# Zeudon/sound-event-localization-detection

Hardware: AMD Instinct MI355X
Metric: training clips/sec (4ch FOA 60s@24kHz) (higher is better)
Workload: dtype bf16; 1 GPU; crnn FOA 4-ch 60s clips, bs=32 windows (BASELINE configs[1]); parallelism=dp1

## Files before the change

### include/seld_hip.h

```cpp
#ifndef SELD_HIP_H_
#define SELD_HIP_H_

#include <stdint.h>

#ifdef __cplusplus
extern "C" {
#endif

int seld_init(int device);
int seld_shutdown(void);
int seld_version(void);
const char* seld_last_error(void);

int seld_set_mel_filterbank(const float* fb_host);

int seld_set_window(const float* window_host);

int seld_default_tables(float* window960, float* fb481x64, int* mel_b0_64, float* mel_wd_24x64,
                        float* mel_wu_24x64);

int64_t seld_num_frames(int64_t L);

int seld_logmel_f32(const float* pcm, int64_t N, int64_t C, int64_t L, float* out, int layout, void* stream);
int seld_logmel_i16(const int16_t* pcm, int64_t N, int64_t C, int64_t L, float* out, int layout, void* stream);
// ... 82 lines not shown
int seld_sum_chunks(const void* partial, int in_is_bf16, int64_t chunks, int64_t count, void* out, int out_is_bf16,
                    void* stream);

int64_t seld_column_sums_blocks(int64_t rows, int64_t n_cols);
int seld_column_sums(const void* g, int in_is_bf16, int64_t rows, int64_t n_cols, float* partial, void* out, int out_is_bf16,
                     void* stream);

int seld_multi_sum_chunks(const void* const* partial, void* const* out, const int64_t* counts, const int32_t* chunks,
                          const int32_t* flags, int count, void* stream);
int seld_multi_column_sums_scratch(const int64_t* rows, const int64_t* n_cols, int count, int64_t* partial_floats);
int seld_multi_column_sums(const void* const* g, void* const* out, const int64_t* rows, const int64_t* n_cols,
                           const int32_t* flags, int count, float* partial, int64_t partial_floats, void* stream);

int seld_gru_dwhh_finish(const void* p_gi, const void* p_n, int in_is_bf16, int64_t chunks, int64_t H, void* dw_hh,
                         int out_is_bf16, void* stream);

int seld_conv_weight_flip_transpose(const void* w, int elem_bytes, int64_t O, int64_t I, void* wt, void* stream);

int seld_conv3x3_wgrad_supported(int64_t F, int64_t Cin, int64_t Cout);
int64_t seld_conv3x3_wgrad_workspace_floats(int64_t B, int64_t T, int64_t F, int64_t Cin, int64_t Cout);
int seld_conv3x3_wgrad(const void* x, const void* dy, int64_t B, int64_t T, int64_t F, int64_t Cin, int64_t Cout,
                       void* dw, int dw_is_bf16, float* workspace, void* stream);

int64_t seld_conv_tail_workspace_floats(int C);
int seld_conv_tail_forward(const void* x, const void* residual, int is_bf16, int64_t rows, int C, int pool,
                           const float* weight, const float* bias, float* running_mean, float* running_var,
                           float momentum, float eps, int training, void* y, float* mean_invstd, float* scale_shift,
                           float* workspace, void* stream);
int seld_conv_tail_backward(const void* x, const void* residual, const void* dy, int is_bf16, int64_t rows, int C,
                            int pool, const float* mean_invstd, const float* scale_shift, void* dx, void* dresidual,
                            float* dweight, float* dbias, float* workspace, void* stream);

int seld_dwconv1d(const void* x, int is_bf16, const float* weight, const float* bias, int64_t B, int64_t T, int D, int K,
                  int flip_taps, void* y, void* stream);
int64_t seld_dwconv1d_wgrad_rows(int64_t B, int64_t T);
int seld_dwconv1d_wgrad(const void* x, const void* dy, int is_bf16, int64_t B, int64_t T, int D, int K, float* partial,
                        void* stream);

int64_t seld_gru_tile_rows(void);
int seld_gru_forward(const void* gi, int is_bf16, const void* w_hh_bf16, const float* b_hn, int64_t B,
                     int64_t T, int64_t H, void* y, void* saved_tile, void* stream);

int seld_gru_backward(const void* dy_tile, const void* saved_tile, const void* y, int is_bf16,
                      const void* w_hh_t_bf16, int64_t tiles, int64_t T, int64_t H, void* dg_tile, float* dbias,
                      void* stream);

// ... 19 lines not shown
```

### sound-event-localization-detection_amd/config.py

```python
from pathlib import Path

_SR = 24000


class Config:
    BASE_PATH = Path(__file__).parent
    AUDIO_PATH = BASE_PATH / "foa_dev"
    METADATA_PATH = BASE_PATH / "metadata_dev"
    OUTPUT_PATH = BASE_PATH / "outputs"
    CHECKPOINT_PATH = BASE_PATH / "checkpoints"

    USE_FULL_DATASET = True
    TRAIN_AUDIO_FILE = "fold3_room21_mix001.wav"
    TRAIN_META_FILE = "fold3_room21_mix001.csv"
    TEST_AUDIO_FILE = "fold4_room23_mix001.wav"
    TEST_META_FILE = "fold4_room23_mix001.csv"

    STARSS22_CLASSES = dict(enumerate((
        "Female speech, woman speaking", "Male speech, man speaking", "Clapping", "Telephone",
        "Laughter", "Domestic sounds", "Walk, footsteps", "Door, open or close", "Music",
        "Musical instrument", "Water tap, faucet", "Bell", "Knock", "Background")))

    MODEL_TYPE = "resnet_conformer"
    NUM_CLASSES = 14
# ... 31 lines not shown
    MIN_DELTA = 1e-4

    SAVE_EVERY_N_EPOCHS = 5
    KEEP_LAST_N_CHECKPOINTS = 3

    SPECTROGRAM_N_FFT = int(0.04 * _SR)
    SPECTROGRAM_HOP_LENGTH = int(0.02 * _SR)
    N_MELS = 64
    SR = _SR

    WINDOW_LENGTH = int(5 * _SR)
    HOP_LENGTH = int(1 * _SR)

    I = None
    J = None
    GRID_CELL_DEGREES = 10

    AMP_DTYPE = "bf16"
    CHANNELS_LAST = True
    FUSED_LOSS = True
    FUSED_CONV_TAIL = True
    CONV_DGRAD_AS_FORWARD = True
    FUSED_CONV_WGRAD = True
    FUSED_DWCONV = "auto"
    CONV1X1_AS_GEMM = True
    FUSED_QKV = True
    FUSED_LAYERNORM = True
    OVERLAP_WEIGHT_GRADS = True
    FUSED_GRU = True
    DEVICE_FEED = True
    MASTER_WEIGHTS = True
    FUSED_ADAM_KERNEL = True
    GRAPH_STEP = True
    OVERLAP_ALLREDUCE = True
    ALLREDUCE_CUT_LEVELS = 2
    GRAD_REDUCE_DTYPE = "param"
    TUNED_GEMMS = True
    DDP_BUCKET_MB = 8
    SYNC_BATCHNORM = False
    SEED = None
    FEATURE_SET = "logmel"
    FEATURE_CACHE_DIR = None
    THREE_TERM_LOSS = False
    GAUSSIAN_AUGMENT = False
    GAUSSIAN_SIGMA_AZIMUTH = 5.0
    GAUSSIAN_SIGMA_ELEVATION = 5.0
# ... 18 lines not shown
```

### sound-event-localization-detection_amd/model_crnn.py

```python
import torch
import torch.nn as nn
import torch.nn.functional as F

from seld_layernorm import run_head
from seld_linear import SeldLinear
from seld_rnn import SeldGRU


class _Conv3x3(torch.autograd.Function):

    enabled = True
    fused_wgrad = True

    @staticmethod
    def forward(ctx, x, weight):
        cdt = torch.get_autocast_dtype("cuda") if torch.is_autocast_enabled() else x.dtype
        with torch.autocast(device_type="cuda", enabled=False):
            xc, wc = x.to(cdt), weight.to(cdt)
            y = F.conv2d(xc, wc, padding=1)
        ctx.save_for_backward(xc, wc)
        ctx.dtypes = (x.dtype, weight.dtype)
        ctx.after_cut = bool(x.is_leaf and x.requires_grad)
        return y

# ... 36 lines not shown
        return dx, dw if dw.dtype == w_dtype else dw.to(w_dtype)


def conv3x3(c, x):
    if (x.is_cuda and _Conv3x3.enabled and c.kernel_size == (3, 3) and c.stride == (1, 1) and c.padding == (1, 1)
            and c.dilation == (1, 1) and c.groups == 1 and c.bias is None and c.padding_mode == "zeros"
            and x.is_contiguous(memory_format=torch.channels_last) and torch.is_grad_enabled()
            and (x.requires_grad or c.weight.requires_grad)):
        return _Conv3x3.apply(x, c.weight)
    return c(x)


class ConvBlock(nn.Module):

    def __init__(self, in_channels, out_channels, kernel_size=(3, 3), stride=(1, 1), padding=(1, 1), pool_size=None):
        super().__init__()
        self.conv = nn.Conv2d(in_channels, out_channels, kernel_size=kernel_size, stride=stride,
                              padding=padding, bias=False)
        self.bn = nn.BatchNorm2d(out_channels)
        self.act = nn.ReLU(inplace=True)
        self.pool = nn.MaxPool2d(pool_size) if pool_size else None

    def forward(self, x):
        x = conv3x3(self.conv, x)
        if x.is_cuda:
            import seld_convtail
            if seld_convtail.applicable(self, x):
                return seld_convtail.conv_tail(self, x)
        x = self.act(self.bn(x))
        return x if self.pool is None else self.pool(x)


def build_cnn_encoder(n_channels, n_mels, cnn_channels, max_pools=4):
    blocks = nn.ModuleList()
    channels, freq = n_channels, n_mels
    for depth, width in enumerate(cnn_channels):
        pool = (1, 2) if depth < max_pools else None
        blocks.append(ConvBlock(channels, width, pool_size=pool))
        channels = width
        if pool:
            freq //= pool[1]
    return blocks, channels, freq


def run_cnn_blocks(blocks, x, inner_cut=True):
    x = x.permute(0, 2, 1, 3)
# ... 59 lines not shown
```

### sound-event-localization-detection_amd/seld_native.py

```python
from __future__ import annotations

import ctypes
import os
import threading
from pathlib import Path

import torch

_HERE = Path(__file__).resolve().parent
LIB_PATH = Path(os.environ["SELD_HIP_LIB"]).resolve() if os.environ.get("SELD_HIP_LIB") else _HERE / "libseld_hip.so"

N_FFT = 960
HOP = 480
N_BINS = 481
N_MELS = 64

_lock = threading.Lock()
_lib = None
_initialised_devices = set()

_i64 = ctypes.c_int64
_int = ctypes.c_int
_ptr = ctypes.c_void_p

# ... 44 lines not shown
    lib.seld_smr_loss_workspace_bytes.argtypes = [_i64, _i64]
    lib.seld_smr_loss.argtypes = [_ptr, _int, _ptr, _ptr, _i64, _int, _int, _int, ctypes.c_float, ctypes.c_float,
                                  ctypes.c_float, _ptr, _ptr, _ptr, _ptr]
    lib.seld_multi_cast.argtypes = [_ptr, _ptr, _ptr, _int, _int, _ptr]
    lib.seld_stream_delay.argtypes = [_i64, _ptr]
    lib.seld_gru_fold_bias.argtypes = [_ptr, _ptr, _i64, _ptr, _int, _ptr, _ptr]
    lib.seld_gru_bias_grads.argtypes = [_ptr, _i64, _i64, _ptr, _ptr, _ptr]
    lib.seld_sum_chunks.argtypes = [_ptr, _int, _i64, _i64, _ptr, _int, _ptr]
    lib.seld_gru_dwhh_finish.argtypes = [_ptr, _ptr, _int, _i64, _i64, _ptr, _int, _ptr]
    lib.seld_column_sums.argtypes = [_ptr, _int, _i64, _i64, _ptr, _ptr, _int, _ptr]
    _pp, _pi64, _pi32 = ctypes.POINTER(ctypes.c_void_p), ctypes.POINTER(ctypes.c_int64), ctypes.POINTER(ctypes.c_int32)
    _f = ctypes.c_float
    lib.seld_multi_adam.argtypes = [_pp, _pi32, _pp, _pp, _pp, _pp, _pi64, _int, _ptr, _ptr, _f, _f, _f, _f, _f, _ptr]
    lib.seld_multi_sum_chunks.argtypes = [_pp, _pp, _pi64, _pi32, _pi32, _int, _ptr]
    lib.seld_multi_column_sums_scratch.argtypes = [_pi64, _pi64, _int, _pi64]
    lib.seld_multi_column_sums.argtypes = [_pp, _pp, _pi64, _pi64, _pi32, _int, _ptr, _i64, _ptr]
    lib.seld_column_sums_blocks.argtypes = [_i64, _i64]
    lib.seld_column_sums_blocks.restype = ctypes.c_int64
    lib.seld_conv_weight_flip_transpose.argtypes = [_ptr, _int, _i64, _i64, _ptr, _ptr]
    lib.seld_conv3x3_wgrad_supported.argtypes = [_i64, _i64, _i64]
    lib.seld_conv3x3_wgrad_workspace_floats.restype = _i64
    lib.seld_conv3x3_wgrad_workspace_floats.argtypes = [_i64, _i64, _i64, _i64, _i64]
    lib.seld_conv3x3_wgrad.argtypes = [_ptr, _ptr, _i64, _i64, _i64, _i64, _i64, _ptr, _int, _ptr, _ptr]
    lib.seld_layernorm_supported.argtypes = [_i64]
    lib.seld_layernorm_workspace_floats.restype = _i64
    lib.seld_layernorm_workspace_floats.argtypes = [_i64, _i64]
    lib.seld_layernorm_forward.argtypes = [_ptr, _int, _i64, _i64, _ptr, _ptr, ctypes.c_float, _int, _ptr, _ptr, _ptr]
    lib.seld_layernorm_backward.argtypes = [_ptr, _ptr, _int, _i64, _i64, _ptr, _ptr, _ptr, _int, _ptr, _ptr, _ptr,
                                            _ptr, _ptr]
    lib.seld_conv_tail_workspace_floats.restype = _i64
    lib.seld_conv_tail_workspace_floats.argtypes = [_int]
    lib.seld_conv_tail_forward.argtypes = [_ptr, _ptr, _int, _i64, _int, _int, _ptr, _ptr, _ptr, _ptr, ctypes.c_float,
                                           ctypes.c_float, _int, _ptr, _ptr, _ptr, _ptr, _ptr]
    lib.seld_conv_tail_backward.argtypes = [_ptr, _ptr, _ptr, _int, _i64, _int, _int, _ptr, _ptr, _ptr, _ptr, _ptr, _ptr,
                                            _ptr, _ptr]
    lib.seld_dwconv1d.argtypes = [_ptr, _int, _ptr, _ptr, _i64, _i64, _int, _int, _int, _ptr, _ptr]
    lib.seld_dwconv1d_wgrad.argtypes = [_ptr, _ptr, _int, _i64, _i64, _int, _int, _ptr, _ptr]
    lib.seld_dwconv1d_wgrad_rows.argtypes = [_i64, _i64]
    lib.seld_dwconv1d_wgrad_rows.restype = ctypes.c_int64
    lib.seld_gru_to_tile.argtypes = [_ptr, _int, _i64, _i64, _int, _ptr, _ptr]
    lib.seld_gru_from_pair_tile.argtypes = [_ptr, _int, _i64, _i64, _ptr, _ptr, _ptr]
    lib.seld_gru_previous_state.argtypes = [_ptr, _int, _i64, _i64, _ptr, _ptr]
    lib.seld_gru_tile_rows.restype = _i64
    lib.seld_gru_tile_rows.argtypes = []
    lib.seld_gru_forward.argtypes = [_ptr, _int, _ptr, _ptr, _i64, _i64, _i64, _ptr, _ptr, _ptr]
    lib.seld_gru_backward.argtypes = [_ptr, _ptr, _ptr, _int, _ptr, _i64, _i64, _i64, _ptr, _ptr, _ptr]
# ... 794 lines not shown
            and dy.dtype == torch.bfloat16 and tuple(w.shape[2:]) == (3, 3)):
        return False
    b, cin, t, f = x.shape
    if tuple(dy.shape) != (b, w.shape[0], t, f) or w.shape[1] != cin:
        return False
    if not (x.is_contiguous(memory_format=torch.channels_last) and dy.is_contiguous(memory_format=torch.channels_last)
            and w.is_contiguous(memory_format=torch.channels_last)):
        return False
    return bool(load_library().seld_conv3x3_wgrad_supported(f, cin, w.shape[0]))


def conv3x3_wgrad(x: torch.Tensor, dy: torch.Tensor, dw: torch.Tensor) -> torch.Tensor:
    if not conv3x3_wgrad_applicable(x, dy, dw) or dw.dtype not in (torch.float32, torch.bfloat16):
        raise SeldNativeError("conv3x3_wgrad: unsupported shapes, dtypes or layouts")
    b, cin, t, f = x.shape
    cout = dy.shape[1]
    with _device_guard(ensure_init(x.device)):
        lib = load_library()
        ws = torch.empty(int(lib.seld_conv3x3_wgrad_workspace_floats(b, t, f, cin, cout)), dtype=torch.float32,
                         device=x.device)
        check(lib.seld_conv3x3_wgrad(_p(x), _p(dy), b, t, f, cin, cout, _p(dw), _is_bf16(dw), _p(ws),
                                     _stream_ptr(x.device)), "seld_conv3x3_wgrad")
    return dw



def _prep_pcm(pcm):
    squeeze = pcm.dim() == 2
    if squeeze:
        pcm = pcm.unsqueeze(0)
    if pcm.dim() != 3 or not pcm.is_cuda or pcm.dtype not in (torch.float32, torch.int16):
        raise SeldNativeError("pcm must be a GPU tensor [N, C, L] (or [C, L]) of float32 or int16")
    return pcm.contiguous(), squeeze


def stft(pcm: torch.Tensor) -> torch.Tensor:
    pcm, squeeze = _prep_pcm(pcm)
    n, c, length = pcm.shape
    index = ensure_init(pcm.device)
    out = torch.empty((n, c, num_frames(length), N_BINS, 2), dtype=torch.float32, device=pcm.device)
    fn = load_library().seld_stft_f32 if pcm.dtype == torch.float32 else load_library().seld_stft_i16
    with _device_guard(index):
        check(fn(_p(pcm), n, c, length, _p(out), _stream_ptr(pcm.device)), "seld_stft")
    spec = torch.view_as_complex(out)
    return spec[0] if squeeze else spec

# ... 51 lines not shown
```

### sound-event-localization-detection_amd/trainer.py

```python
import gc
import logging
import os
import random
from contextlib import nullcontext
from datetime import datetime
from pathlib import Path

import numpy as np
import torch
import torch.distributed as dist
from torch.utils.data import DataLoader, RandomSampler, SequentialSampler
from tqdm import tqdm

from config import Config
from dataset import SELDDataset
from loss import SMRSELDLoss
from model import SMRSELDWithCSPDarkNet
from model_conformer import SELD_Conformer
from model_crnn import SELD_CRNN
from resnet50_model import SELD_ResNet50_Conformer
from seld_rnn import SeldGRU
from utils import get_local_rank, get_rank, get_world_size, safe_torch_load
from visualization import plot_loss_curves, visualize_grid_predictions, visualize_loss_components

# ... 21 lines not shown
        logger.info("Initializing ResNet50-Conformer model...")
        return SELD_ResNet50_Conformer(n_mels=config.N_MELS, conf_d_model=config.RESNET_CONF_D_MODEL,
                                       conf_n_heads=config.RESNET_CONF_N_HEADS,
                                       conf_n_layers=config.RESNET_CONF_N_LAYERS,
                                       dropout=config.RESNET_DROPOUT, **common)
    logger.info("Initializing CSPDarkNet (CNN) model...")
    return SMRSELDWithCSPDarkNet(use_small=use_small_model, **common)


def prepare_model_for_device(model, device):
    model = model.to(device)
    if device.type == "cuda" and getattr(config, "CHANNELS_LAST", True):
        model = model.to(memory_format=torch.channels_last)
    SeldGRU.fused_enabled = bool(getattr(config, "FUSED_GRU", True))
    if device.type == "cuda":
        import seld_convtail
        import seld_gru
        seld_convtail.enabled = bool(getattr(config, "FUSED_CONV_TAIL", True))
        import model_crnn
        model_crnn._Conv3x3.enabled = bool(getattr(config, "CONV_DGRAD_AS_FORWARD", True)) and \
            os.environ.get("SELD_CONV_AS_FWD", "1") != "0"
        model_crnn._Conv3x3.fused_wgrad = bool(getattr(config, "FUSED_CONV_WGRAD", True)) and \
            os.environ.get("SELD_CONV_WGRAD", "1") != "0"
        if os.environ.get("SELD_DWCONV") is None:
            import seld_dwconv
            seld_dwconv.enabled = getattr(config, "FUSED_DWCONV", "auto")
            if seld_dwconv.enabled == "auto" and graph_step_enabled(device):
                seld_dwconv.enabled = True
        import seld_layernorm
        seld_layernorm.enabled = bool(getattr(config, "FUSED_LAYERNORM", True)) and \
            os.environ.get("SELD_LAYERNORM", "1") != "0"
        if os.environ.get("SELD_OVERLAP") is None:
            import seld_overlap
            seld_overlap.enabled = bool(getattr(config, "OVERLAP_WEIGHT_GRADS", True))
        import seld_linear
        seld_linear.conv1x1_as_gemm = bool(getattr(config, "CONV1X1_AS_GEMM", True)) and \
            os.environ.get("SELD_CONV1X1_GEMM", "1") != "0"
        import model_conformer
        model_conformer.MultiHeadSelfAttention.fused_qkv = bool(getattr(config, "FUSED_QKV", True)) and \
            os.environ.get("SELD_FUSED_QKV", "1") != "0"
        for module in model.modules():
            if isinstance(module, SeldGRU) and SeldGRU.fused_enabled:
                seld_gru.pack_parameters(module)
            if isinstance(module, model_conformer.MultiHeadSelfAttention):
                module.pack_parameters()
        if os.environ.get("SELD_CUT_LEVELS") is None:
# ... 696 lines not shown
```

Measured before the change: 154.8 clips/s.

## Fuse first CRNN conv block (conv3x3+BN+ReLU+pool) into MFMA kernels

Adds a dedicated HIP path for the first CRNN conv block, which has 4 input channels and 64 output channels. The forward pass recomputes the 3x3 convolution with MFMA in a stats pass and then an apply pass, so the full-resolution pre-pool activation is never written to memory. The backward pass likewise fuses dgrad-free weight gradients and BN gradients, since the input needs no grad. The cost is recomputing the conv twice per pass and extra launches for the statistics reduction.

```diff
diff --git a/include/seld_hip.h b/include/seld_hip.h
--- a/include/seld_hip.h
+++ b/include/seld_hip.h
@@ -128,6 +128,18 @@
 int seld_conv3x3_wgrad(const void* x, const void* dy, int64_t B, int64_t T, int64_t F, int64_t Cin, int64_t Cout,
                        void* dw, int dw_is_bf16, float* workspace, void* stream);
 
+int seld_convfirst_supported(int64_t F, int64_t Cin, int64_t Cout);
+int64_t seld_convfirst_workspace_floats(int backward);
+int seld_convfirst_forward(const void* in, const void* w, int w_is_bf16, int64_t w_sco, int64_t w_sci, int64_t w_sr,
+                           int64_t w_ss, int64_t B, int64_t T, int64_t F, const float* bn_weight, const float* bn_bias,
+                           float* running_mean, float* running_var, float momentum, float eps, void* y,
+                           float* mean_invstd, float* scale_shift, float* workspace, int phases, void* stream);
+int seld_convfirst_backward(const void* in, const void* w, int w_is_bf16, int64_t w_sco, int64_t w_sci, int64_t w_sr,
+                            int64_t w_ss, const void* dy, int64_t B, int64_t T, int64_t F, const float* mean_invstd,
+                            const float* scale_shift, void* dw, int dw_is_bf16, int64_t dw_sco, int64_t dw_sci,
+                            int64_t dw_sr, int64_t dw_ss, float* dgamma, float* dbeta, float* workspace, int phases,
+                            void* stream);
+
 int64_t seld_conv_tail_workspace_floats(int C);
 int seld_conv_tail_forward(const void* x, const void* residual, int is_bf16, int64_t rows, int C, int pool,
                            const float* weight, const float* bias, float* running_mean, float* running_var,
diff --git a/sound-event-localization-detection_amd/config.py b/sound-event-localization-detection_amd/config.py
--- a/sound-event-localization-detection_amd/config.py
+++ b/sound-event-localization-detection_amd/config.py
@@ -77,6 +77,7 @@
     FUSED_CONV_TAIL = True
     CONV_DGRAD_AS_FORWARD = True
     FUSED_CONV_WGRAD = True
+    FUSED_FIRST_BLOCK = True
     FUSED_DWCONV = "auto"
     CONV1X1_AS_GEMM = True
     FUSED_QKV = True
diff --git a/sound-event-localization-detection_amd/csrc/convfirst.hip b/sound-event-localization-detection_amd/csrc/convfirst.hip
--- /dev/null
+++ b/sound-event-localization-detection_amd/csrc/convfirst.hip
@@ -0,0 +1,711 @@
+#include <hip/hip_bf16.h>
+
+#include "seld_common.h"
+
+namespace seld {
+
+namespace {
+
+typedef __attribute__((ext_vector_type(8))) __bf16 bf16x8;
+typedef __attribute__((ext_vector_type(2))) __bf16 bf16x2;
+typedef __attribute__((ext_vector_type(2))) float f32x2;
+typedef __attribute__((ext_vector_type(4))) float f32x4;
+typedef __attribute__((ext_vector_type(4))) unsigned u32x4;
+typedef __attribute__((ext_vector_type(2))) short s16x2;
+typedef __attribute__((ext_vector_type(4))) short s16x4;
+typedef __attribute__((ext_vector_type(8))) short s16x8;
+typedef __attribute__((address_space(3))) s16x4 lds_s16x4;
+
+constexpr int kCfThreads = 256;
+constexpr int kCfPos = 256;
+constexpr int kCfTiles = kCfPos / 16;
+constexpr int kCfCout = 64;
+constexpr int kCfCin = 4;
+constexpr int kCfK = 36;
+constexpr int kCfMaxGroups = 512;
+constexpr int kCfImage = 3 * 258;
+constexpr int kCfStage = 3;
+constexpr int kCfSumThreads = 256;
+constexpr int kCfSumRows = 16;
+
+struct CfGeom {
+  int T, logF, chunks_per_clip, chunks;
+  long rows;
+};
+
+struct CfWeights {
+  const void* w;
+  int is_bf16;
+  int packed;
+  long sco, sci, sr, ss;
+};
+
+__device__ __forceinline__ unsigned pack_bf16_pair(float lo, float hi) {
+  const f32x2 v = {lo, hi};
+  return __builtin_bit_cast(unsigned, __builtin_convertvector(v, bf16x2));
+}
+__device__ __forceinline__ float round_bf16(float z) { return __uint_as_float(pack_bf16_pair(z, 0.0f) << 16); }
+__device__ __forceinline__ float bf16_lo(unsigned w) { return __uint_as_float(w << 16); }
+__device__ __forceinline__ float bf16_hi(unsigned w) { return __uint_as_float(w & 0xffff0000u); }
+
+__device__ __forceinline__ float cf_weight(const CfWeights& w, int co, int tap, int ci) {
+  const long i = co * w.sco + ci * w.sci + (tap / 3) * w.sr + (tap % 3) * w.ss;
+  if (w.is_bf16) return __uint_as_float(static_cast<unsigned>(static_cast<const unsigned short*>(w.w)[i]) << 16);
+  return round_bf16(static_cast<const float*>(w.w)[i]);
+}
+
+__device__ __forceinline__ void cf_load_weights(const CfWeights& w, int lane, bf16x8 (&wb)[4][2]) {
+  const int g = lane >> 4, c = lane & 15;
+  if (w.packed) {
+#pragma unroll
+    for (int nt = 0; nt < 4; ++nt) {
+      const uint2* const row = reinterpret_cast<const uint2*>(static_cast<const unsigned short*>(w.w) + (4 * c + nt) * kCfK);
+      const uint2 lo = row[2 * g], hi = row[2 * g + 1];
+      uint2 last = row[8];
+      if (g != 0) last = make_uint2(0u, 0u);
+      const u32x4 p0 = {lo.x, lo.y, hi.x, hi.y}, p1 = {last.x, last.y, 0u, 0u};
+      wb[nt][0] = __builtin_bit_cast(bf16x8, p0);
+      wb[nt][1] = __builtin_bit_cast(bf16x8, p1);
+    }
+    return;
+  }
+#pragma unroll
+  for (int nt = 0; nt < 4; ++nt) {
+    const int co = 4 * c + nt;
+    float v0[8], v1[8];
+#pragma unroll
+    for (int e = 0; e < 8; ++e) {
+      v0[e] = cf_weight(w, co, 2 * g + (e >> 2), e & 3);
+      v1[e] = (g == 0 && e < 4) ? cf_weight(w, co, 8, e & 3) : 0.0f;
+    }
+    const u32x4 p0 = {pack_bf16_pair(v0[0], v0[1]), pack_bf16_pair(v0[2], v0[3]), pack_bf16_pair(v0[4], v0[5]),
+                      pack_bf16_pair(v0[6], v0[7])};
+    const u32x4 p1 = {pack_bf16_pair(v1[0], v1[1]), pack_bf16_pair(v1[2], v1[3]), pack_bf16_pair(v1[4], v1[5]),
+                      pack_bf16_pair(v1[6], v1[7])};
+    wb[nt][0] = __builtin_bit_cast(bf16x8, p0);
+    wb[nt][1] = __builtin_bit_cast(bf16x8, p1);
+  }
+}
+
+__device__ __forceinline__ int cf_tap_shift(int tap, int W) { return (tap / 3 - 1) * W + tap % 3 - 1; }
+
+__device__ __forceinline__ int cf_image_row(int pos, int logF) {
+  const int F = 1 << logF;
+  return ((pos >> logF) + 1) * (F + 2) + (pos & (F - 1)) + 1;
+}
+
+struct CfLane {
+  int xr[kCfTiles / 4];
+  int row[kCfTiles / 4];
+  int pooled[kCfTiles / 4];
+  int sh0, sh1, sh8;
+  bool g0;
+};
+
+__device__ __forceinline__ CfLane cf_lane(int logF, int lane, int wave) {
+  CfLane ln;
+  const int W = (1 << logF) + 2, g = lane >> 4;
+#pragma unroll
+  for (int i = 0; i < kCfTiles / 4; ++i) {
+    const int pos = (wave + 4 * i) * 16;
+    ln.xr[i] = cf_image_row(pos + (lane & 15), logF);
+    ln.row[i] = pos >> logF;
+    ln.pooled[i] = ((pos + 4 * g) >> 1) * kCfCout + 4 * (lane & 15);
+  }
+  ln.sh0 = cf_tap_shift(2 * g, W);
+  ln.sh1 = cf_tap_shift(2 * g + 1, W);
+  ln.sh8 = W + 1;
+  ln.g0 = g == 0;
+  return ln;
+}
+
+__device__ __forceinline__ void cf_conv_tile(const uint2* img, const CfLane& ln, int i, const bf16x8 (&wb)[4][2],
+                                             unsigned (&xp)[4][2]) {
+  const int xr = ln.xr[i];
+  const uint2 t0 = img[xr + ln.sh0], t1 = img[xr + ln.sh1];
+  uint2 t8 = img[xr + ln.sh8];
+  if (!ln.g0) t8 = make_uint2(0u, 0u);
+  const u32x4 p0 = {t0.x, t0.y, t1.x, t1.y}, p1 = {t8.x, t8.y, 0u, 0u};
+  const bf16x8 a0 = __builtin_bit_cast(bf16x8, p0), a1 = __builtin_bit_cast(bf16x8, p1);
+#pragma unroll
+  for (int nt = 0; nt < 4; ++nt) {
+    f32x4 acc = {0.0f, 0.0f, 0.0f, 0.0f};
+    acc = __builtin_amdgcn_mfma_f32_16x16x32_bf16(a0, wb[nt][0], acc, 0, 0, 0);
+    acc = __builtin_amdgcn_mfma_f32_16x16x32_bf16(a1, wb[nt][1], acc, 0, 0, 0);
+    xp[nt][0] = pack_bf16_pair(acc[0], acc[1]);
+    xp[nt][1] = pack_bf16_pair(acc[2], acc[3]);
+  }
+}
+
+__device__ __forceinline__ bf16x8 cf_operand(const unsigned (&t0)[2], const unsigned (&t1)[2]) {
+  const u32x4 v = {t0[0], t0[1], t1[0], t1[1]};
+  return __builtin_bit_cast(bf16x8, v);
+}
+__device__ __forceinline__ bf16x8 cf_ones() {
+  const u32x4 v = {0x3f803f80u, 0x3f803f80u, 0x3f803f80u, 0x3f803f80u};
+  return __builtin_bit_cast(bf16x8, v);
+}
+
+__device__ __forceinline__ unsigned cf_relu_pair(unsigned p) {
+  const s16x2 v = __builtin_bit_cast(s16x2, p), zero = {0, 0};
+  return __builtin_bit_cast(unsigned, __builtin_elementwise_max(v, zero));
+}
+
+__device__ __forceinline__ unsigned cf_activate(unsigned xpair, float a, float b) {
+  return cf_relu_pair(pack_bf16_pair(fmaf(bf16_lo(xpair), a, b), fmaf(bf16_hi(xpair), a, b)));
+}
+
+struct CfChunk {
+  int b, t0;
+};
+
+__device__ __forceinline__ CfChunk cf_chunk(const CfGeom& gm, int chunk) {
+  CfChunk c;
+  c.b = chunk / gm.chunks_per_clip;
+  c.t0 = (chunk - c.b * gm.chunks_per_clip) * (kCfPos >> gm.logF);
+  return c;
+}
+
+__device__ __forceinline__ void cf_load_image(const uint2* in, const CfGeom& gm, const CfChunk& c, uint2 (&r)[kCfStage]) {
+  const int pieces = ((kCfPos >> gm.logF) + 2) << gm.logF;
+#pragma unroll
+  for (int i = 0; i < kCfStage; ++i) {
+    const int p = threadIdx.x + i * kCfThreads;
+    const int t = c.t0 - 1 + (p >> gm.logF);
+    r[i] = make_uint2(0u, 0u);
+    if (p < pieces && t >= 0 && t < gm.T)
+      r[i] = in[((static_cast<long>(c.b) * gm.T + t) << gm.logF) + (p & ((1 << gm.logF) - 1))];
+  }
+}
+
+__device__ __forceinline__ void cf_store_image(uint2* img, const CfGeom& gm, const uint2 (&r)[kCfStage]) {
+  const int F = 1 << gm.logF, pieces = ((kCfPos >> gm.logF) + 2) << gm.logF;
+#pragma unroll
+  for (int i = 0; i < kCfStage; ++i) {
+    const int p = threadIdx.x + i * kCfThreads;
+    if (p < pieces) img[(p >> gm.logF) * (F + 2) + (p & (F - 1)) + 1] = r[i];
+  }
+}
+
+__device__ __forceinline__ bool cf_tile_valid(const CfGeom& gm, const CfChunk& c, const CfLane& ln, int i) {
+  return c.t0 + ln.row[i] < gm.T;
+}
+
+__device__ __forceinline__ long cf_pooled_base(const CfGeom& gm, const CfChunk& c) {
+  return (((static_cast<long>(c.b) * gm.T + c.t0) << gm.logF) >> 1) * kCfCout;
+}
+
+__device__ __forceinline__ float cf_pick(const f32x4& v, int j) {
+  return j == 0 ? v[0] : j == 1 ? v[1] : j == 2 ? v[2] : v[3];
+}
+
+__device__ __forceinline__ void cf_block_partials(const f32x4 (&colsum)[4], const f32x4 (&diag)[4], float* part ,
+                                                  float* __restrict__ partials, int nrows) {
+  const int tid = threadIdx.x, lane = tid & 63, wave = tid >> 6, g = lane >> 4, c = lane & 15;
+#pragma unroll
+  for (int nt = 0; nt < 4; ++nt) {
+    if (g == 0) part[wave * 128 + 4 * c + nt] = colsum[nt][0];
+    if (g == (c >> 2)) part[wave * 128 + 64 + 4 * c + nt] = cf_pick(diag[nt], c & 3);
+  }
+  __syncthreads();
+  if (tid < 2 * kCfCout) {
+    const int s = tid >> 6, ch = tid & 63;
+    const float sum = ((part[tid] + part[128 + tid]) + part[256 + tid]) + part[384 + tid];
+    partials[(static_cast<long>(s) * nrows + blockIdx.x) * kCfCout + ch] = sum;
+  }
+}
+
+constexpr int kCfFinalThreads = 256;
+
+__device__ __forceinline__ void cf_final_sums(const float* __restrict__ partials, int nrows, double* red ) {
+  const int tid = threadIdx.x, item = tid & 15, s = item >> 3, ch = blockIdx.x * 8 + (item & 7), rg = tid >> 4;
+  double sum = 0.0;
+#pragma unroll 8
+  for (int r = rg; r < nrows; r += 16) sum += static_cast<double>(partials[(static_cast<long>(s) * nrows + r) * kCfCout + ch]);
+  red[rg * 16 + item] = sum;
+  __syncthreads();
+  if (tid < 16) {
+    for (int k = 1; k < 16; ++k) sum += red[k * 16 + tid];
+    red[tid] = sum;
+  }
+  __syncthreads();
+}
+
+__global__ __launch_bounds__(kCfFinalThreads) void convfirst_stats_final_kernel(
+    const float* __restrict__ partials, int nrows, long rows, const float* __restrict__ weight,
+    const float* __restrict__ bias, float* __restrict__ running_mean, float* __restrict__ running_var, float momentum,
+    float eps, float* __restrict__ mean_invstd, float* __restrict__ scale_shift) {
+  __shared__ double red[16 * 16];
+  cf_final_sums(partials, nrows, red);
+  if (threadIdx.x < 8) {
+    const int ch = blockIdx.x * 8 + threadIdx.x;
+    const double n = static_cast<double>(rows);
+    const double mean = red[threadIdx.x] / n;
+    double var = red[8 + threadIdx.x] / n - mean * mean;
+    if (var < 0.0) var = 0.0;
+    const double unbiased = rows > 1 ? var * n / (n - 1.0) : var;
+    running_mean[ch] = static_cast<float>((1.0 - momentum) * running_mean[ch] + momentum * mean);
+    running_var[ch] = static_cast<float>((1.0 - momentum) * running_var[ch] + momentum * unbiased);
+    const float meanf = static_cast<float>(mean);
+    const float invstd = static_cast<float>(1.0 / sqrt(var + static_cast<double>(eps)));
+    const float a = weight[ch] * invstd;
+    mean_invstd[ch] = meanf;
+    mean_invstd[kCfCout + ch] = invstd;
+    scale_shift[ch] = a;
+    scale_shift[kCfCout + ch] = bias[ch] - meanf * a;
+  }
+}
+
+__global__ __launch_bounds__(kCfFinalThreads) void convfirst_bwd_final_kernel(
+    const float* __restrict__ partials, int nrows, long rows, const float* __restrict__ mean_invstd,
+    const float* __restrict__ scale_shift, float* __restrict__ dgamma, float* __restrict__ dbeta,
+    float* __restrict__ coef ) {
+  __shared__ double red[16 * 16];
+  cf_final_sums(partials, nrows, red);
+  if (threadIdx.x < 8) {
+    const int ch = blockIdx.x * 8 + threadIdx.x;
+    const double invstd = mean_invstd[kCfCout + ch], mean = mean_invstd[ch], a = scale_shift[ch];
+    const double s_dz = red[threadIdx.x], s_dzx = (red[8 + threadIdx.x] - mean * s_dz) * invstd;
+    const double n = static_cast<double>(rows);
+    dbeta[ch] = static_cast<float>(s_dz);
+    dgamma[ch] = static_cast<float>(s_dzx);
+    const double q = -a * (s_dzx / n) * invstd;
+    coef[ch] = static_cast<float>(-a * (s_dz / n) - q * mean);
+    coef[kCfCout + ch] = static_cast<float>(q);
+  }
+}
+
+#define SELD_CF_PROLOGUE()                                                                   \
+  const int tid = threadIdx.x, lane = tid & 63, wave = tid >> 6;                             \
+  const uint2* const in2 = static_cast<const uint2*>(in);                                    \
+  for (int i = tid; i < kCfImage; i += kCfThreads) img[i] = make_uint2(0u, 0u);              \
+  const CfLane ln = cf_lane(gm.logF, lane, wave)
+
+__global__ __launch_bounds__(kCfThreads, 2) void convfirst_stats_kernel(const void* __restrict__ in, CfWeights w, CfGeom gm,
+                                                                        float* __restrict__ partials) {
+  __shared__ uint2 img[kCfImage];
+  __shared__ float part[4 * 128];
+  SELD_CF_PROLOGUE();
+  f32x4 colsum[4], diag[4];
+#pragma unroll
+  for (int nt = 0; nt < 4; ++nt) colsum[nt] = diag[nt] = f32x4{0.0f, 0.0f, 0.0f, 0.0f};
+  const bf16x8 ones = cf_ones();
+  uint2 rin[kCfStage];
+  int chunk = blockIdx.x;
+  if (chunk < gm.chunks) cf_load_image(in2, gm, cf_chunk(gm, chunk), rin);
+  bf16x8 wb[4][2];
+  cf_load_weights(w, lane, wb);
+  for (; chunk < gm.chunks; chunk += gridDim.x) {
+    const CfChunk c = cf_chunk(gm, chunk);
+    __syncthreads();
+    cf_store_image(img, gm, rin);
+    __syncthreads();
+    if (chunk + static_cast<int>(gridDim.x) < gm.chunks) cf_load_image(in2, gm, cf_chunk(gm, chunk + gridDim.x), rin);
+#pragma unroll
+    for (int h = 0; h < 2; ++h) {
+      unsigned xp[2][4][2] = {};
+#pragma unroll
+      for (int u = 0; u < 2; ++u)
+        if (cf_tile_valid(gm, c, ln, 2 * h + u)) cf_conv_tile(img, ln, 2 * h + u, wb, xp[u]);
+#pragma unroll
+      for (int nt = 0; nt < 4; ++nt) {
+        const bf16x8 x = cf_operand(xp[0][nt], xp[1][nt]);
+        colsum[nt] = __builtin_amdgcn_mfma_f32_16x16x32_bf16(ones, x, colsum[nt], 0, 0, 0);
+        diag[nt] = __builtin_amdgcn_mfma_f32_16x16x32_bf16(x, x, diag[nt], 0, 0, 0);
+      }
+    }
+  }
+  cf_block_partials(colsum, diag, part, partials, gridDim.x);
+}
+
+__global__ __launch_bounds__(kCfThreads, 2) void convfirst_apply_kernel(const void* __restrict__ in, CfWeights w, CfGeom gm,
+                                                                        const float* __restrict__ scale_shift,
+                                                                        unsigned short* __restrict__ y) {
+  __shared__ uint2 img[kCfImage];
+  SELD_CF_PROLOGUE();
+  uint2 rin[kCfStage];
+  int chunk = blockIdx.x;
+  if (chunk < gm.chunks) cf_load_image(in2, gm, cf_chunk(gm, chunk), rin);
+  bf16x8 wb[4][2];
+  cf_load_weights(w, lane, wb);
+  float a[4], b[4];
+#pragma unroll
+  for (int nt = 0; nt < 4; ++nt) {
+    a[nt] = scale_shift[4 * (lane & 15) + nt];
+    b[nt] = scale_shift[kCfCout + 4 * (lane & 15) + nt];
+  }
+  for (; chunk < gm.chunks; chunk += gridDim.x) {
+    const CfChunk c = cf_chunk(gm, chunk);
+    __syncthreads();
+    cf_store_image(img, gm, rin);
+    __syncthreads();
+    if (chunk + static_cast<int>(gridDim.x) < gm.chunks) cf_load_image(in2, gm, cf_chunk(gm, chunk + gridDim.x), rin);
+#pragma unroll
+    for (int i = 0; i < kCfTiles / 4; ++i) {
+      if (!cf_tile_valid(gm, c, ln, i)) continue;
+      unsigned xp[4][2];
+      cf_conv_tile(img, ln, i, wb, xp);
+      const long o = cf_pooled_base(gm, c) + ln.pooled[i];
+#pragma unroll
+      for (int jp = 0; jp < 2; ++jp) {
+        unsigned m[4];
+#pragma unroll
+        for (int nt = 0; nt < 4; ++nt) {
+          const unsigned z = cf_activate(xp[nt][jp], a[nt], b[nt]);
+          m[nt] = max(z & 0xffffu, z >> 16);
+        }
+        *reinterpret_cast<uint2*>(y + o + jp * kCfCout) = make_uint2(m[0] | (m[1] << 16), m[2] | (m[3] << 16));
+      }
+    }
+  }
+}
+
+__device__ __forceinline__ void cf_load_dy(const unsigned short* dy, const CfGeom& gm, const CfChunk& c, const CfLane& ln,
+                                           uint2 (&r)[kCfTiles / 4][2]) {
+  const unsigned short* const base = dy + cf_pooled_base(gm, c);
+#pragma unroll
+  for (int i = 0; i < kCfTiles / 4; ++i) {
+    const bool valid = cf_tile_valid(gm, c, ln, i);
+    const unsigned short* const o = base + ln.pooled[i];
+#pragma unroll
+    for (int jp = 0; jp < 2; ++jp) {
+      r[i][jp] = make_uint2(0u, 0u);
+      if (valid) r[i][jp] = *reinterpret_cast<const uint2*>(o + jp * kCfCout);
+    }
+  }
+}
+
+__global__ __launch_bounds__(kCfThreads, 2) void convfirst_bwd_reduce_kernel(
+    const void* __restrict__ in, CfWeights w, CfGeom gm, const unsigned short* __restrict__ dy,
+    const float* __restrict__ scale_shift, float* __restrict__ partials) {
+  __shared__ uint2 img[kCfImage];
+  __shared__ float part[4 * 128];
+  SELD_CF_PROLOGUE();
+  float a[4], b[4];
+  f32x4 colsum[4], diag[4];
+#pragma unroll
+  for (int nt = 0; nt < 4; ++nt) {
+    a[nt] = scale_shift[4 * (lane & 15) + nt];
+    b[nt] = scale_shift[kCfCout + 4 * (lane & 15) + nt];
+    colsum[nt] = diag[nt] = f32x4{0.0f, 0.0f, 0.0f, 0.0f};
+  }
+  const bf16x8 ones = cf_ones();
+  uint2 rin[kCfStage], rdy[kCfTiles / 4][2];
+  int chunk = blockIdx.x;
+  if (chunk < gm.chunks) {
+    cf_load_image(in2, gm, cf_chunk(gm, chunk), rin);
+    cf_load_dy(dy, gm, cf_chunk(gm, chunk), ln, rdy);
+  }
+  bf16x8 wb[4][2];
+  cf_load_weights(w, lane, wb);
+  for (; chunk < gm.chunks; chunk += gridDim.x) {
+    const CfChunk c = cf_chunk(gm, chunk);
+    __syncthreads();
+    cf_store_image(img, gm, rin);
+    uint2 g2[kCfTiles / 4][2];
+#pragma unroll
+    for (int i = 0; i < kCfTiles / 4; ++i) {
+      g2[i][0] = rdy[i][0];
+      g2[i][1] = rdy[i][1];
+    }
+    __syncthreads();
+    if (chunk + static_cast<int>(gridDim.x) < gm.chunks) {
+      cf_load_image(in2, gm, cf_chunk(gm, chunk + gridDim.x), rin);
+      cf_load_dy(dy, gm, cf_chunk(gm, chunk + gridDim.x), ln, rdy);
+    }
+#pragma unroll
+    for (int h = 0; h < 2; ++h) {
+      unsigned xp[2][4][2] = {}, dz[2][4][2] = {};
+#pragma unroll
+      for (int u = 0; u < 2; ++u) {
+        if (!cf_tile_valid(gm, c, ln, 2 * h + u)) continue;
+        cf_conv_tile(img, ln, 2 * h + u, wb, xp[u]);
+#pragma unroll
+        for (int jp = 0; jp < 2; ++jp) {
+          const uint2 gw = g2[2 * h + u][jp];
+#pragma unroll
+          for (int nt = 0; nt < 4; ++nt) {
+            const unsigned z = cf_activate(xp[u][nt][jp], a[nt], b[nt]);
+            const unsigned word = nt < 2 ? gw.x : gw.y;
+            const unsigned to_lo = (nt & 1) ? word >> 16 : word & 0xffffu;
+            const unsigned to_hi = (nt & 1) ? word & 0xffff0000u : word << 16;
+            dz[u][nt][jp] = z == 0u ? 0u : ((z >> 16) > (z & 0xffffu) ? to_hi : to_lo);
+          }
+        }
+      }
+#pragma unroll
+      for (int nt = 0; nt < 4; ++nt) {
+        const bf16x8 x = cf_operand(xp[0][nt], xp[1][nt]), d = cf_operand(dz[0][nt], dz[1][nt]);
+        colsum[nt] = __builtin_amdgcn_mfma_f32_16x16x32_bf16(ones, d, colsum[nt], 0, 0, 0);
+        diag[nt] = __builtin_amdgcn_mfma_f32_16x16x32_bf16(d, x, diag[nt], 0, 0, 0);
+      }
+    }
+  }
+  cf_block_partials(colsum, diag, part, partials, gridDim.x);
+}
+
+__device__ __forceinline__ s16x4 cf_tr_read(const unsigned short* base, int offset_shorts) {
+  return __builtin_amdgcn_ds_read_tr16_b64_v4i16((lds_s16x4*)(base + offset_shorts));
+}
+__device__ __forceinline__ bf16x8 cf_join(s16x4 lo, s16x4 hi) {
+  const s16x8 v = __builtin_shufflevector(lo, hi, 0, 1, 2, 3, 4, 5, 6, 7);
+  return __builtin_bit_cast(bf16x8, v);
+}
+
+__global__ __launch_bounds__(kCfThreads, 2) void convfirst_wgrad_kernel(
+    const void* __restrict__ in, CfWeights w, CfGeom gm, const unsigned short* __restrict__ dy,
+    const float* __restrict__ scale_shift, const float* __restrict__ coef, float* __restrict__ slots) {
+  __shared__ uint2 img[kCfImage];
+  SELD_CF_PROLOGUE();
+  uint2 rin[kCfStage], rdy[kCfTiles / 4][2];
+  int chunk = blockIdx.x;
+  if (chunk < gm.chunks) {
+    cf_load_image(in2, gm, cf_chunk(gm, chunk), rin);
+    cf_load_dy(dy, gm, cf_chunk(gm, chunk), ln, rdy);
+  }
+  bf16x8 wb[4][2];
+  cf_load_weights(w, lane, wb);
+  float a[4], b[4], p[4], q[4];
+#pragma unroll
+  for (int nt = 0; nt < 4; ++nt) {
+    const int ch = 4 * (lane & 15) + nt;
+    a[nt] = scale_shift[ch];
+    b[nt] = scale_shift[kCfCout + ch];
+    p[nt] = coef[ch];
+    q[nt] = coef[kCfCout + ch];
+  }
+  const int W = (1 << gm.logF) + 2, g = lane >> 4, qq = (lane >> 2) & 3, pp = lane & 3;
+  int tap_shift[3];
+#pragma unroll
+  for (int nb = 0; nb < 3; ++nb) tap_shift[nb] = cf_tap_shift(min(4 * nb + pp, 8), W);
+  int xb[kCfTiles / 4];
+#pragma unroll
+  for (int i = 0; i < kCfTiles / 4; ++i) xb[i] = cf_image_row((wave + 4 * i) * 16 + 4 * g + qq, gm.logF);
+  f32x4 acc[4][3];
+#pragma unroll
+  for (int nt = 0; nt < 4; ++nt)
+#pragma unroll
+    for (int nb = 0; nb < 3; ++nb) acc[nt][nb] = f32x4{0.0f, 0.0f, 0.0f, 0.0f};
+  const unsigned short* const imgs = reinterpret_cast<const unsigned short*>(img);
+
+  for (; chunk < gm.chunks; chunk += gridDim.x) {
+    const CfChunk c = cf_chunk(gm, chunk);
+    __syncthreads();
+    cf_store_image(img, gm, rin);
+    uint2 g2[kCfTiles / 4][2];
+#pragma unroll
+    for (int i = 0; i < kCfTiles / 4; ++i) {
+      g2[i][0] = rdy[i][0];
+      g2[i][1] = rdy[i][1];
+    }
+    __syncthreads();
+    if (chunk + static_cast<int>(gridDim.x) < gm.chunks) {
+      cf_load_image(in2, gm, cf_chunk(gm, chunk + gridDim.x), rin);
+      cf_load_dy(dy, gm, cf_chunk(gm, chunk + gridDim.x), ln, rdy);
+    }
+#pragma unroll
+    for (int h = 0; h < 2; ++h) {
+      unsigned dxp[2][4][2] = {};
+#pragma unroll
+      for (int u = 0; u < 2; ++u) {
+        if (!cf_tile_valid(gm, c, ln, 2 * h + u)) continue;
+        unsigned xp[4][2];
+        cf_conv_tile(img, ln, 2 * h + u, wb, xp);
+#pragma unroll
+        for (int jp = 0; jp < 2; ++jp) {
+          const uint2 gw = g2[2 * h + u][jp];
+#pragma unroll
+          for (int nt = 0; nt < 4; ++nt) {
+            const unsigned z = cf_activate(xp[nt][jp], a[nt], b[nt]);
+            const unsigned word = nt < 2 ? gw.x : gw.y;
+            const float gv = (nt & 1) ? bf16_hi(word) : bf16_lo(word);
+            const bool pass = z != 0u, second = (z >> 16) > (z & 0xffffu);
+            const float g0 = (pass && !second) ? gv : 0.0f, g1 = (pass && second) ? gv : 0.0f;
+            const float d0 = fmaf(a[nt], g0, fmaf(q[nt], bf16_lo(xp[nt][jp]), p[nt]));
+            const float d1 = fmaf(a[nt], g1, fmaf(q[nt], bf16_hi(xp[nt][jp]), p[nt]));
+            dxp[u][nt][jp] = pack_bf16_pair(d0, d1);
+          }
+        }
+      }
+      const int xr0 = xb[2 * h], xr1 = xb[2 * h + 1];
+      bf16x8 bf[3];
+#pragma unroll
+      for (int nb = 0; nb < 3; ++nb)
+        bf[nb] = cf_join(cf_tr_read(imgs, (xr0 + tap_shift[nb]) * kCfCin), cf_tr_read(imgs, (xr1 + tap_shift[nb]) * kCfCin));
+#pragma unroll
+      for (int nt = 0; nt < 4; ++nt) {
+        const bf16x8 af = cf_operand(dxp[0][nt], dxp[1][nt]);
+#pragma unroll
+        for (int nb = 0; nb < 3; ++nb) acc[nt][nb] = __builtin_amdgcn_mfma_f32_16x16x32_bf16(af, bf[nb], acc[nt][nb], 0, 0, 0);
+      }
+    }
+  }
+  __syncthreads();
+  __shared__ float tile[kCfCout * kCfK];
+  for (int wv = 0; wv < 4; ++wv) {
+    if (wave == wv) {
+#pragma unroll
+      for (int nt = 0; nt < 4; ++nt)
+#pragma unroll
+        for (int nb = 0; nb < 3; ++nb) {
+          const int n = nb * 16 + (lane & 15);
+          if (n < kCfK)
+#pragma unroll
+            for (int j = 0; j < 4; ++j) {
+              float* const e = tile + (4 * (4 * g + j) + nt) * kCfK + n;
+              *e = wv == 0 ? acc[nt][nb][j] : *e + acc[nt][nb][j];
+            }
+        }
+    }
+    __syncthreads();
+  }
+  float* const slot = slots + static_cast<long>(blockIdx.x) * kCfCout * kCfK;
+  for (int i = tid; i < kCfCout * kCfK; i += kCfThreads) slot[i] = tile[i];
+}
+
+__global__ __launch_bounds__(kCfSumThreads) void convfirst_wgrad_sum_kernel(const float* __restrict__ slots, int nslots,
+                                                                            void* __restrict__ dw, int dw_is_bf16, long sco,
+                                                                            long sci, long sr, long ss) {
+  constexpr int kCols = kCfSumThreads / kCfSumRows;
+  constexpr int kCount = kCfCout * kCfK;
+  __shared__ float4 part[kCfSumRows][kCols];
+  const int col = threadIdx.x % kCols, row = threadIdx.x / kCols;
+  const int i = (blockIdx.x * kCols + col) * 4;
+  float4 s = make_float4(0.0f, 0.0f, 0.0f, 0.0f);
+  if (i < kCount)
+    for (int k = row; k < nslots; k += kCfSumRows) {
+      const float4 v = *reinterpret_cast<const float4*>(slots + static_cast<long>(k) * kCount + i);
+      s.x += v.x; s.y += v.y; s.z += v.z; s.w += v.w;
+    }
+  part[row][col] = s;
+  __syncthreads();
+  if (row != 0 || i >= kCount) return;
+#pragma unroll
+  for (int r = 1; r < kCfSumRows; ++r) {
+    const float4 v = part[r][col];
+    s.x += v.x; s.y += v.y; s.z += v.z; s.w += v.w;
+  }
+  const int co = i / kCfK, tap = (i - co * kCfK) >> 2;
+  const long o = co * sco + (tap / 3) * sr + (tap % 3) * ss;
+  const float v[4] = {s.x, s.y, s.z, s.w};
+#pragma unroll
+  for (int ci = 0; ci < kCfCin; ++ci) {
+    if (dw_is_bf16) static_cast<unsigned short*>(dw)[o + ci * sci] = static_cast<unsigned short>(pack_bf16_pair(v[ci], 0.0f) & 0xffffu);
+    else static_cast<float*>(dw)[o + ci * sci] = v[ci];
+  }
+}
+
+#undef SELD_CF_PROLOGUE
+
+bool cf_supported(int64_t F, int64_t Cin, int64_t Cout) {
+  return Cin == kCfCin && Cout == kCfCout && (F == 16 || F == 32 || F == 64 || F == 128 || F == 256);
+}
+
+int cf_geometry(const char* who, int64_t B, int64_t T, int64_t F, CfGeom* gm) {
+  if (B <= 0 || T <= 0) return fail(kErrInvalidArgument, std::string(who) + ": B and T must be positive");
+  if (!cf_supported(F, kCfCin, kCfCout)) return fail(kErrUnsupported, std::string(who) + ": F must be 16, 32, 64, 128 or 256");
+  int logF = 4;
+  while ((1 << logF) < F) ++logF;
+  const int tc = kCfPos >> logF;
+  const int64_t per_clip = (T + tc - 1) / tc;
+  if (B * per_clip > (1 << 30) || B * T * F > (1LL << 40)) return fail(kErrUnsupported, std::string(who) + ": tensor too large");
+  gm->T = static_cast<int>(T);
+  gm->logF = logF;
+  gm->chunks_per_clip = static_cast<int>(per_clip);
+  gm->chunks = static_cast<int>(B * per_clip);
+  gm->rows = B * T * F;
+  return kOk;
+}
+
+int cf_groups(const DeviceState* st, const CfGeom& gm) {
+  int groups = 2 * (st->num_cus > 0 ? st->num_cus : 256);
+  if (groups > kCfMaxGroups) groups = kCfMaxGroups;
+  return groups < gm.chunks ? groups : gm.chunks;
+}
+
+bool cf_aligned(const void* p, uintptr_t a) { return (reinterpret_cast<uintptr_t>(p) & (a - 1)) == 0; }
+
+int cf_packed(const void* w, int is_bf16, int64_t sco, int64_t sci, int64_t sr, int64_t ss) {
+  return is_bf16 && sci == 1 && ss == kCfCin && sr == 3 * kCfCin && sco == kCfK && cf_aligned(w, 8) ? 1 : 0;
+}
+
+}
+
+}
+
+extern "C" {
+
+int seld_convfirst_supported(int64_t F, int64_t Cin, int64_t Cout) { return seld::cf_supported(F, Cin, Cout) ? 1 : 0; }
+
+int64_t seld_convfirst_workspace_floats(int backward) {
+  using namespace seld;
+  const int64_t partials = 2LL * kCfMaxGroups * kCfCout;
+  return backward ? partials + static_cast<int64_t>(kCfMaxGroups) * kCfCout * kCfK + 2 * kCfCout : partials;
+}
+
+int seld_convfirst_forward(const void* in, const void* w, int w_is_bf16, int64_t w_sco, int64_t w_sci, int64_t w_sr,
+                           int64_t w_ss, int64_t B, int64_t T, int64_t F, const float* bn_weight, const float* bn_bias,
+                           float* running_mean, float* running_var, float momentum, float eps, void* y,
+                           float* mean_invstd, float* scale_shift, float* workspace, int phases, void* stream_) {
+  using namespace seld;
+  const DeviceState* st = current_state();
+  if (!st) return kErrNotInitialised;
+  CfGeom gm;
+  if (int rc = cf_geometry("seld_convfirst_forward", B, T, F, &gm)) return rc;
+  if (!in || !w || !bn_weight || !bn_bias || !running_mean || !running_var || !y || !mean_invstd || !scale_shift || !workspace)
+    return fail(kErrInvalidArgument, "seld_convfirst_forward: null pointer");
+  if (!cf_aligned(in, 8) || !cf_aligned(y, 8) || !cf_aligned(workspace, 16))
+    return fail(kErrInvalidArgument, "seld_convfirst_forward: in / y 8-byte, workspace 16-byte aligned required");
+  hipStream_t stream = static_cast<hipStream_t>(stream_);
+  const CfWeights cw{w, w_is_bf16, cf_packed(w, w_is_bf16, w_sco, w_sci, w_sr, w_ss), static_cast<long>(w_sco), static_cast<long>(w_sci), static_cast<long>(w_sr), static_cast<long>(w_ss)};
+  const int groups = cf_groups(st, gm);
+  if (phases & 1)
+    hipLaunchKernelGGL(convfirst_stats_kernel, dim3(groups), dim3(kCfThreads), 0, stream, in, cw, gm, workspace);
+  if (phases & 2) {
+    hipLaunchKernelGGL(convfirst_stats_final_kernel, dim3(kCfCout / 8), dim3(kCfFinalThreads), 0, stream, workspace, groups,
+                       gm.rows, bn_weight, bn_bias, running_mean, running_var, momentum, eps, mean_invstd, scale_shift);
+    hipLaunchKernelGGL(convfirst_apply_kernel, dim3(groups), dim3(kCfThreads), 0, stream, in, cw, gm, scale_shift,
+                       static_cast<unsigned short*>(y));
+  }
+  SELD_HIP_TRY(hipGetLastError());
+  return kOk;
+}
+
+int seld_convfirst_backward(const void* in, const void* w, int w_is_bf16, int64_t w_sco, int64_t w_sci, int64_t w_sr,
+                            int64_t w_ss, const void* dy, int64_t B, int64_t T, int64_t F, const float* mean_invstd,
+                            const float* scale_shift, void* dw, int dw_is_bf16, int64_t dw_sco, int64_t dw_sci,
+                            int64_t dw_sr, int64_t dw_ss, float* dgamma, float* dbeta, float* workspace, int phases,
+                            void* stream_) {
+  using namespace seld;
+  const DeviceState* st = current_state();
+  if (!st) return kErrNotInitialised;
+  CfGeom gm;
+  if (int rc = cf_geometry("seld_convfirst_backward", B, T, F, &gm)) return rc;
+  if (!in || !w || !dy || !mean_invstd || !scale_shift || !dw || !dgamma || !dbeta || !workspace)
+    return fail(kErrInvalidArgument, "seld_convfirst_backward: null pointer");
+  if (!cf_aligned(in, 8) || !cf_aligned(dy, 8) || !cf_aligned(workspace, 16))
+    return fail(kErrInvalidArgument, "seld_convfirst_backward: in / dy 8-byte, workspace 16-byte aligned required");
+  hipStream_t stream = static_cast<hipStream_t>(stream_);
+  const CfWeights cw{w, w_is_bf16, cf_packed(w, w_is_bf16, w_sco, w_sci, w_sr, w_ss), static_cast<long>(w_sco), static_cast<long>(w_sci), static_cast<long>(w_sr), static_cast<long>(w_ss)};
+  const int groups = cf_groups(st, gm);
+  float* const slots = workspace + 2L * kCfMaxGroups * kCfCout;
+  float* const coef = slots + static_cast<long>(kCfMaxGroups) * kCfCout * kCfK;
+  const unsigned short* const g = static_cast<const unsigned short*>(dy);
+  if (phases & 1)
+    hipLaunchKernelGGL(convfirst_bwd_reduce_kernel, dim3(groups), dim3(kCfThreads), 0, stream, in, cw, gm, g, scale_shift,
+                       workspace);
+  if (phases & 2) {
+    hipLaunchKernelGGL(convfirst_bwd_final_kernel, dim3(kCfCout / 8), dim3(kCfFinalThreads), 0, stream, workspace, groups,
+                       gm.rows, mean_invstd, scale_shift, dgamma, dbeta, coef);
+    hipLaunchKernelGGL(convfirst_wgrad_kernel, dim3(groups), dim3(kCfThreads), 0, stream, in, cw, gm, g, scale_shift, coef,
+                       slots);
+    constexpr int kCols = kCfSumThreads / kCfSumRows;
+    hipLaunchKernelGGL(convfirst_wgrad_sum_kernel, dim3((kCfCout * kCfK / 4 + kCols - 1) / kCols), dim3(kCfSumThreads), 0,
+                       stream, slots, groups, dw, dw_is_bf16, static_cast<long>(dw_sco), static_cast<long>(dw_sci),
+                       static_cast<long>(dw_sr), static_cast<long>(dw_ss));
+  }
+  SELD_HIP_TRY(hipGetLastError());
+  return kOk;
+}
+
+}
diff --git a/sound-event-localization-detection_amd/model_crnn.py b/sound-event-localization-detection_amd/model_crnn.py
--- a/sound-event-localization-detection_amd/model_crnn.py
+++ b/sound-event-localization-detection_amd/model_crnn.py
@@ -82,6 +82,10 @@
         self.pool = nn.MaxPool2d(pool_size) if pool_size else None
 
     def forward(self, x):
+        if x.is_cuda and self.conv.in_channels <= 8:
+            import seld_convfirst
+            if seld_convfirst.applicable(self, x):
+                return seld_convfirst.first_block(self, x)
         x = conv3x3(self.conv, x)
         if x.is_cuda:
             import seld_convtail
diff --git a/sound-event-localization-detection_amd/seld_convfirst.py b/sound-event-localization-detection_amd/seld_convfirst.py
--- /dev/null
+++ b/sound-event-localization-detection_amd/seld_convfirst.py
@@ -0,0 +1,57 @@
+import torch
+import torch.nn as nn
+
+import seld_convtail
+import seld_native
+
+enabled = True
+
+
+def applicable(block, x):
+    if not (enabled and seld_convtail.enabled and x.is_cuda and x.dim() == 4 and torch.is_grad_enabled()
+            and not x.requires_grad):
+        return False
+    import model_crnn
+    conv, bn, pool = block.conv, block.bn, block.pool
+    if not (model_crnn._Conv3x3.enabled and type(conv) is nn.Conv2d and conv.kernel_size == (3, 3)
+            and conv.stride == (1, 1) and conv.padding == (1, 1) and conv.dilation == (1, 1) and conv.groups == 1
+            and conv.bias is None and conv.padding_mode == "zeros" and conv.weight.requires_grad):
+        return False
+    if not (type(bn) is nn.BatchNorm2d and bn.training and bn.affine and bn.track_running_stats
+            and bn.momentum is not None and bn.weight.dtype == torch.float32 and bn.weight.requires_grad
+            and bn.bias.requires_grad):
+        return False
+    if type(pool) is not nn.MaxPool2d:
+        return False
+    k = pool.kernel_size if isinstance(pool.kernel_size, tuple) else (pool.kernel_size,) * 2
+    s = pool.stride if isinstance(pool.stride, tuple) else (pool.stride,) * 2
+    if tuple(k) != (1, 2) or tuple(s) != (1, 2) or pool.padding not in (0, (0, 0)) or pool.ceil_mode \
+            or pool.dilation not in (1, (1, 1)):
+        return False
+    return seld_native.convfirst_applicable(x, conv.weight)
+
+
+class _ConvFirst(torch.autograd.Function):
+    @staticmethod
+    def forward(ctx, x, conv_weight, bn_weight, bn_bias, running_mean, running_var, momentum, eps):
+        y, mean_invstd, scale_shift = seld_native.convfirst_forward(x, conv_weight, bn_weight, bn_bias, running_mean,
+                                                                    running_var, momentum, eps)
+        ctx.save_for_backward(x, conv_weight, mean_invstd, scale_shift)
+        return y
+
+    @staticmethod
+    def backward(ctx, dy):
+        x, conv_weight, mean_invstd, scale_shift = ctx.saved_tensors
+        dw = torch.empty_like(conv_weight)
+        dw, dgamma, dbeta = seld_native.convfirst_backward(x, conv_weight, dy, mean_invstd, scale_shift, dw)
+        return None, dw, dgamma, dbeta, None, None, None, None
+
+
+def first_block(block, x):
+    bn = block.bn
+    if seld_convtail._collected is not None:
+        seld_convtail._collected.append(bn.num_batches_tracked)
+    else:
+        bn.num_batches_tracked.add_(1)
+    return _ConvFirst.apply(x, block.conv.weight, bn.weight, bn.bias, bn.running_mean, bn.running_var, bn.momentum,
+                            bn.eps)
diff --git a/sound-event-localization-detection_amd/seld_native.py b/sound-event-localization-detection_amd/seld_native.py
--- a/sound-event-localization-detection_amd/seld_native.py
+++ b/sound-event-localization-detection_amd/seld_native.py
@@ -90,6 +90,13 @@
     lib.seld_conv3x3_wgrad_workspace_floats.restype = _i64
     lib.seld_conv3x3_wgrad_workspace_floats.argtypes = [_i64, _i64, _i64, _i64, _i64]
     lib.seld_conv3x3_wgrad.argtypes = [_ptr, _ptr, _i64, _i64, _i64, _i64, _i64, _ptr, _int, _ptr, _ptr]
+    lib.seld_convfirst_supported.argtypes = [_i64, _i64, _i64]
+    lib.seld_convfirst_workspace_floats.restype = _i64
+    lib.seld_convfirst_workspace_floats.argtypes = [_int]
+    lib.seld_convfirst_forward.argtypes = [_ptr, _ptr, _int, _i64, _i64, _i64, _i64, _i64, _i64, _i64, _ptr, _ptr, _ptr, _ptr,
+                                           ctypes.c_float, ctypes.c_float, _ptr, _ptr, _ptr, _ptr, _int, _ptr]
+    lib.seld_convfirst_backward.argtypes = [_ptr, _ptr, _int, _i64, _i64, _i64, _i64, _ptr, _i64, _i64, _i64, _ptr, _ptr,
+                                            _ptr, _int, _i64, _i64, _i64, _i64, _ptr, _ptr, _ptr, _int, _ptr]
     lib.seld_layernorm_supported.argtypes = [_i64]
     lib.seld_layernorm_workspace_floats.restype = _i64
     lib.seld_layernorm_workspace_floats.argtypes = [_i64, _i64]
@@ -930,6 +937,51 @@
         check(lib.seld_conv3x3_wgrad(_p(x), _p(dy), b, t, f, cin, cout, _p(dw), _is_bf16(dw), _p(ws),
                                      _stream_ptr(x.device)), "seld_conv3x3_wgrad")
     return dw
+
+
+
+def convfirst_applicable(x: torch.Tensor, w: torch.Tensor) -> bool:
+    if not (x.is_cuda and x.dim() == 4 and w.dim() == 4 and x.dtype == torch.bfloat16
+            and w.dtype in (torch.float32, torch.bfloat16) and tuple(w.shape[2:]) == (3, 3) and w.shape[1] == x.shape[1]
+            and x.is_contiguous(memory_format=torch.channels_last)):
+        return False
+    return bool(load_library().seld_convfirst_supported(x.shape[3], x.shape[1], w.shape[0]))
+
+
+def convfirst_forward(x, w, bn_weight, bn_bias, running_mean, running_var, momentum, eps, phases=3):
+    if not convfirst_applicable(x, w):
+        raise SeldNativeError("convfirst: unsupported shapes, dtypes or layouts")
+    b, _, t, f = x.shape
+    index = ensure_init(x.device)
+    y = torch.empty((b, w.shape[0], t, f // 2), dtype=x.dtype, device=x.device, memory_format=torch.channels_last)
+    stats = torch.empty((2, 2, w.shape[0]), dtype=torch.float32, device=x.device)
+    lib = load_library()
+    ws = torch.empty(int(lib.seld_convfirst_workspace_floats(0)), dtype=torch.float32, device=x.device)
+    with _device_guard(index):
+        check(lib.seld_convfirst_forward(_p(x), _p(w), _is_bf16(w), *w.stride(), b, t, f, _p(bn_weight), _p(bn_bias),
+                                         _p(running_mean), _p(running_var), float(momentum), float(eps), _p(y),
+                                         _p(stats[0]), _p(stats[1]), _p(ws), int(phases), _stream_ptr(x.device)),
+              "seld_convfirst_forward")
+    return y, stats[0], stats[1]
+
+
+def convfirst_backward(x, w, dy, mean_invstd, scale_shift, dw, phases=3):
+    if not convfirst_applicable(x, w) or dw.shape != w.shape or dw.dtype not in (torch.float32, torch.bfloat16):
+        raise SeldNativeError("convfirst: unsupported shapes, dtypes or layouts")
+    b, _, t, f = x.shape
+    if tuple(dy.shape) != (b, w.shape[0], t, f // 2):
+        raise SeldNativeError("convfirst: dy does not match the block's output")
+    if dy.dtype != x.dtype or not dy.is_contiguous(memory_format=torch.channels_last):
+        dy = dy.to(x.dtype).contiguous(memory_format=torch.channels_last)
+    index = ensure_init(x.device)
+    dgb = torch.empty((2, w.shape[0]), dtype=torch.float32, device=x.device)
+    lib = load_library()
+    ws = torch.empty(int(lib.seld_convfirst_workspace_floats(1)), dtype=torch.float32, device=x.device)
+    with _device_guard(index):
+        check(lib.seld_convfirst_backward(_p(x), _p(w), _is_bf16(w), *w.stride(), _p(dy), b, t, f, _p(mean_invstd),
+                                          _p(scale_shift), _p(dw), _is_bf16(dw), *dw.stride(), _p(dgb[0]), _p(dgb[1]),
+                                          _p(ws), int(phases), _stream_ptr(x.device)), "seld_convfirst_backward")
+    return dw, dgb[0], dgb[1]
 
 
 
diff --git a/sound-event-localization-detection_amd/trainer.py b/sound-event-localization-detection_amd/trainer.py
--- a/sound-event-localization-detection_amd/trainer.py
+++ b/sound-event-localization-detection_amd/trainer.py
@@ -67,6 +67,9 @@
             os.environ.get("SELD_CONV_AS_FWD", "1") != "0"
         model_crnn._Conv3x3.fused_wgrad = bool(getattr(config, "FUSED_CONV_WGRAD", True)) and \
             os.environ.get("SELD_CONV_WGRAD", "1") != "0"
+        import seld_convfirst
+        seld_convfirst.enabled = bool(getattr(config, "FUSED_FIRST_BLOCK", True)) and \
+            os.environ.get("SELD_FIRST_BLOCK", "1") != "0"
         if os.environ.get("SELD_DWCONV") is None:
             import seld_dwconv
             seld_dwconv.enabled = getattr(config, "FUSED_DWCONV", "auto")
```

New measurement: 159.5 clips/s (median of 6 runs). +3.0%, better.
